# ming024/FastSpeech2

Measured on AMD Instinct MI355X. Metric: mel-frames/sec (train, 80-bin), higher is better.
Workload: dtype bf16; 1 GPU; BASELINE configs[1]: LJSpeech train, 4+4 FFT layers d=256 2 heads, 80-bin mel, batch=48/GPU, L=128 phonemes, T=925 frames, fwd+loss+bwd+clip+Adam, dropout on, fp32 master weights; global_batch=48, parallelism=dp1, hip_graph=False, side_stream_wgrad=True, windows=1, library=fastspeech2_amd/libfs2hip.so

## Files before the change

fastspeech2_amd/csrc/fs2_attn.hip:

```cpp
#include "fs2_common.h"
#include "fs2_gemm.h"
#include <type_traits>

typedef float f32x16 __attribute__((ext_vector_type(16)));

#define DK 128
__device__ __forceinline__ int swz(int row, int chunk) { return row * 512 + ((chunk ^ (row & 15)) << 4); }
__device__ __forceinline__ int crow(int r, int h2) { return (r & 3) + 8 * (r >> 2) + 4 * h2; }

template <typename T, int NT>
__device__ __forceinline__ void stage_tile(unsigned char* lds, const T* __restrict__ base, long ld, int row0, int nrows_valid,
                                           int tid) {
#pragma unroll
    for (int i = 0; i < 1024 / NT; ++i) {
        int idx = tid + NT * i;
        int r = idx >> 5, c = idx & 31;
        float4 v = make_float4(0.f, 0.f, 0.f, 0.f);
        if (r < nrows_valid) v = ld4<T>(base + (size_t)(row0 + r) * ld + c * 4);
        *reinterpret_cast<float4*>(lds + swz(r, c)) = v;
    }
}

template <typename T>
__global__ void __launch_bounds__(256, 1) attn_fwd_kernel(const T* __restrict__ qkv, long ld, T* __restrict__ ctx, long ldo,
                                                          float* __restrict__ lse, const int32_t* __restrict__ lens, int S,
                                                          int H, float scale) {
    __shared__ __attribute__((aligned(16))) unsigned char sK[32 * 512];
    __shared__ __attribute__((aligned(16))) unsigned char sV[32 * 512];
    const int tid = threadIdx.x, lane = tid & 63, w = tid >> 6, fl = lane & 31, h2 = lane >> 5;
    const int qt = blockIdx.x, h = blockIdx.y, b = blockIdx.z;
    const int len = lens ? min(lens[b], S) : S;
    const int q0 = qt * 128;
    const size_t rowbase = (size_t)b * S;
    T* out = ctx + rowbase * ldo + h * DK;
    float* lse_o = lse + ((size_t)b * H + h) * S;
    if (q0 >= len) {
        for (int i = tid; i < 128 * 32; i += 256) {
            int r = i >> 5, c = (i & 31) * 4;
            if (q0 + r < S) st4<T>(out + (size_t)(q0 + r) * ldo + c, make_float4(0.f, 0.f, 0.f, 0.f));
        }
        if (tid < 128 && q0 + tid < S) lse_o[q0 + tid] = 0.f;
        return;
    }
    const T* Q = qkv + rowbase * ld + h * DK;
    const T* K = qkv + rowbase * ld + (size_t)H * DK + h * DK;
    const T* V = qkv + rowbase * ld + (size_t)2 * H * DK + h * DK;

    const int myq = q0 + w * 32 + fl;
    float qf[64];
#pragma unroll
    for (int u = 0; u < 16; ++u) {
        float4 v = make_float4(0.f, 0.f, 0.f, 0.f);
        if (myq < S) v = ld4<T>(Q + (size_t)myq * ld + h2 * 64 + u * 4);
        qf[u * 4 + 0] = v.x * scale; qf[u * 4 + 1] = v.y * scale; qf[u * 4 + 2] = v.z * scale; qf[u * 4 + 3] = v.w * scale;
    }
    f32x16 o[4];
#pragma unroll
    for (int nb = 0; nb < 4; ++nb)
#pragma unroll
        for (int r = 0; r < 16; ++r) o[nb][r] = 0.f;
    float m = -INFINITY, l = 0.f;

    for (int k0 = 0; k0 < len; k0 += 32) {
        __syncthreads();
        stage_tile<T, 256>(sK, K, ld, k0, min(32, S - k0), tid);
        stage_tile<T, 256>(sV, V, ld, k0, min(32, S - k0), tid);
        __syncthreads();
        f32x16 s;
#pragma unroll
        for (int r = 0; r < 16; ++r) s[r] = 0.f;
#pragma unroll
        for (int u = 0; u < 16; ++u) {
            float4 kf = *reinterpret_cast<const float4*>(sK + swz(fl, h2 * 16 + u));
            s = __builtin_amdgcn_mfma_f32_32x32x2f32(kf.x, qf[u * 4 + 0], s, 0, 0, 0);
            s = __builtin_amdgcn_mfma_f32_32x32x2f32(kf.y, qf[u * 4 + 1], s, 0, 0, 0);
            s = __builtin_amdgcn_mfma_f32_32x32x2f32(kf.z, qf[u * 4 + 2], s, 0, 0, 0);
            s = __builtin_amdgcn_mfma_f32_32x32x2f32(kf.w, qf[u * 4 + 3], s, 0, 0, 0);
        }
        float mx = -INFINITY;
#pragma unroll
        for (int r = 0; r < 16; ++r) {
            if (k0 + crow(r, h2) >= len) s[r] = -INFINITY;
            mx = fmaxf(mx, s[r]);
        }
        mx = fmaxf(mx, __shfl_xor(mx, 32, 64));
        float mn = fmaxf(m, mx);
        float alpha = __expf(m - mn);
        float rs = 0.f;
#pragma unroll
        for (int r = 0; r < 16; ++r) { s[r] = __expf(s[r] - mn); rs += s[r]; }
        rs += __shfl_xor(rs, 32, 64);
        l = l * alpha + rs;
        m = mn;
#pragma unroll
        for (int r = 0; r < 16; ++r) {
            float ar = __shfl(alpha, crow(r, h2), 64);
#pragma unroll
            for (int nb = 0; nb < 4; ++nb) o[nb][r] *= ar;
        }
#pragma unroll
        for (int r = 0; r < 16; ++r) {
            int key = crow(r, h2);
#pragma unroll
            for (int nb = 0; nb < 4; ++nb) {
                int col = nb * 32 + fl;
                float vb = *reinterpret_cast<const float*>(sV + swz(key, col >> 2) + (col & 3) * 4);
                o[nb] = __builtin_amdgcn_mfma_f32_32x32x2f32(s[r], vb, o[nb], 0, 0, 0);
            }
        }
    }
    float linv = l > 0.f ? 1.f / l : 0.f;
    if (h2 == 0 && myq < S) lse_o[myq] = (l > 0.f) ? m + __logf(l) : 0.f;
#pragma unroll
    for (int r = 0; r < 16; ++r) {
        float li = __shfl(linv, crow(r, h2), 64);
        int q = q0 + w * 32 + crow(r, h2);
        if (q < S) {
#pragma unroll
            for (int nb = 0; nb < 4; ++nb) Elem<T>::st(out + (size_t)q * ldo + nb * 32 + fl, o[nb][r] * li);
        }
    }
}


typedef short s16x4 __attribute__((ext_vector_type(4)));
typedef short s16x8 __attribute__((ext_vector_type(8)));
typedef __bf16 bf16x8 __attribute__((ext_vector_type(8)));
typedef __attribute__((address_space(3))) s16x4* lds_s4p;

__device__ __forceinline__ int swzb(int row, int c16) { return row * 256 + ((c16 ^ (((row & 3) << 2) | ((row >> 2) & 3))) << 4); }

template <int NT, int ROWS>
__device__ __forceinline__ void stage_tile_bf16(unsigned char* lds, const bf16_t* __restrict__ base, long ld, int row0,
                                                int nrows_valid, int tid) {
#pragma unroll
    for (int i = 0; i < ROWS * 16 / NT; ++i) {
        int idx = tid + NT * i;
        int r = idx >> 4, c = idx & 15;
        uint4 v = make_uint4(0, 0, 0, 0);
        if (r < nrows_valid) v = *reinterpret_cast<const uint4*>(base + (size_t)(row0 + r) * ld + c * 8);
        *reinterpret_cast<uint4*>(lds + swzb(r, c)) = v;
    }
}
__device__ __forceinline__ bf16x8 frag_k(const unsigned char* lds, int row, int s, int h) {
    return __builtin_bit_cast(bf16x8, *reinterpret_cast<const uint4*>(lds + swzb(row, 2 * s + h)));
}
__device__ __forceinline__ bf16x8 frag_t(const unsigned char* lds, int rowbase, int nb, int lane) {
    int li = lane & 15, g = lane >> 4, h = g >> 1;
    int row = rowbase + 4 * h + (li >> 2);
    int col = nb * 32 + 16 * (g & 1) + 4 * (li & 3);
    int off0 = swzb(row, col >> 3) + ((col & 7) << 1);
    int off1 = swzb(row + 8, col >> 3) + ((col & 7) << 1);
    s16x4 lo = __builtin_amdgcn_ds_read_tr16_b64_v4i16((lds_s4p)(lds + off0));
    s16x4 hi = __builtin_amdgcn_ds_read_tr16_b64_v4i16((lds_s4p)(lds + off1));
    return __builtin_bit_cast(bf16x8, __builtin_shufflevector(lo, hi, 0, 1, 2, 3, 4, 5, 6, 7));
}
__device__ __forceinline__ bf16x8 pack8(const float* p) {
    uint4 v;
    v.x = pack_bf16x2(p[0], p[1]); v.y = pack_bf16x2(p[2], p[3]); v.z = pack_bf16x2(p[4], p[5]); v.w = pack_bf16x2(p[6], p[7]);
    return __builtin_bit_cast(bf16x8, v);
}
__device__ __forceinline__ void load_row_frags(bf16x8* f, const bf16_t* row, int h, bool ok) {
#pragma unroll
    for (int s = 0; s < 8; ++s) {
        uint4 v = make_uint4(0, 0, 0, 0);
        if (ok) v = *reinterpret_cast<const uint4*>(row + 16 * s + 8 * h);
        f[s] = __builtin_bit_cast(bf16x8, v);
    }
}

#define TILE_LD1(t, base, ld_, row0, last_row, I) \
    (t##I) = *reinterpret_cast<const uint4*>((base) + (unsigned)(min((row0) + ((tid + 256 * I) >> 4), (last_row)) * (int)(ld_) + (tid & 15) * 8))
#define TILE_LOAD_REGS(t, base, ld_, row0, last_row) do { TILE_LD1(t, base, ld_, row0, last_row, 0); TILE_LD1(t, base, ld_, row0, last_row, 1); \
    TILE_LD1(t, base, ld_, row0, last_row, 2); TILE_LD1(t, base, ld_, row0, last_row, 3); } while (0)
#define TILE_ST1(lds, t, I) *reinterpret_cast<uint4*>((lds) + swzb((tid + 256 * I) >> 4, tid & 15)) = (t##I)
#define TILE_STORE_REGS(lds, t) do { TILE_ST1(lds, t, 0); TILE_ST1(lds, t, 1); TILE_ST1(lds, t, 2); TILE_ST1(lds, t, 3); } while (0)


#ifdef FS2_DEV
__device__ unsigned long long fs2_attn_stamps[16 * 12];
__device__ int fs2_attn_stamp_kernel = 2;
extern "C" int fs2_dev_attn_stamp_select(int k) { return hipMemcpyToSymbol(HIP_SYMBOL(fs2_attn_stamp_kernel), &k, sizeof(int)) == hipSuccess ? 0 : 1; }
extern "C" int fs2_dev_attn_stamps(unsigned long long* out) {
    return hipMemcpyFromSymbol(out, HIP_SYMBOL(fs2_attn_stamps), sizeof(fs2_attn_stamps)) == hipSuccess ? 0 : 1;
}
#define FS2_STAMP_INIT() const bool fs2_stamp_on = fs2_attn_stamp_kernel == FS2_STAMP_KERNEL && blockIdx.x == 0 && blockIdx.y == 0 && blockIdx.z == 0 && threadIdx.x == 0
#define FS2_STAMP_AT(t0_, i) do { if (fs2_stamp_on && (t0_) < 16 * 64) fs2_attn_stamps[((t0_) >> 6) * 12 + (i)] = __builtin_amdgcn_s_memtime(); } while (0)
#define FS2_STAMP(i) FS2_STAMP_AT(q0, i)
#define FS2_STAMP_RAW(i) do { if (fs2_stamp_on) fs2_attn_stamps[(i)] = __builtin_amdgcn_s_memtime(); } while (0)
#else
#define FS2_STAMP_INIT() do {} while (0)
#define FS2_STAMP_AT(t0_, i) do {} while (0)
#define FS2_STAMP(i) do {} while (0)
#define FS2_STAMP_RAW(i) do {} while (0)
#endif

__device__ __forceinline__ void attn_block_map(int H, int& t, int& h, int& b) {
    const int nt = (int)gridDim.x, nbh = (int)(gridDim.y * gridDim.z);
    const int L = (int)(blockIdx.x + gridDim.x * (blockIdx.y + gridDim.y * blockIdx.z));
    const int G = L / (8 * nt), r = L - G * (8 * nt);
    const int rem = min(8, nbh - 8 * G);
    const int bh = 8 * G + r % rem;
    t = r / rem;
    b = bh / H; h = bh - b * H;
}

template <int IMG, int NTHR> struct FragAddrT {
    unsigned k[8], t0[4], t1[4], st[4];
    int step;
    __device__ __forceinline__ void init(unsigned base, int tid) {
        const int lane = tid & 63, fl = lane & 31, h2 = lane >> 5;
#pragma unroll
        for (int i = 0; i < 8; ++i) k[i] = base + (unsigned)swzb(fl, 2 * i + h2);
        const int li = lane & 15, g = lane >> 4, hh = g >> 1, rr = 4 * hh + (li >> 2);
#pragma unroll
        for (int nb = 0; nb < 4; ++nb) {
            const int col = nb * 32 + 16 * (g & 1) + 4 * (li & 3);
            t0[nb] = base + (unsigned)(swzb(rr, col >> 3) + ((col & 7) << 1));
            t1[nb] = base + (unsigned)(swzb(rr + 8, col >> 3) + ((col & 7) << 1));
        }
#pragma unroll
        for (int I = 0; I < 4; ++I) st[I] = base + (unsigned)(2 * IMG) + (unsigned)swzb((tid + NTHR * I) >> 4, tid & 15);
        step = 2 * IMG;
    }
    __device__ __forceinline__ void flip() {
#pragma unroll
        for (int i = 0; i < 8; ++i) k[i] += (unsigned)step;
#pragma unroll
        for (int nb = 0; nb < 4; ++nb) { t0[nb] += (unsigned)step; t1[nb] += (unsigned)step; }
#pragma unroll
        for (int I = 0; I < 4; ++I) st[I] -= (unsigned)step;
        step = -step;
    }
    __device__ __forceinline__ bf16x8 rk(int img, int blk, int i) const {
        typedef unsigned lds_v4u __attribute__((ext_vector_type(4)));
        typedef __attribute__((address_space(3))) const lds_v4u* lds_u4p;
        return __builtin_bit_cast(bf16x8, *(lds_u4p)(size_t)(k[i] + (unsigned)(img * IMG + blk * 8192)));
    }
    __device__ __forceinline__ bf16x8 rt(int img, int rb, int nb) const {
        s16x4 lo = __builtin_amdgcn_ds_read_tr16_b64_v4i16((lds_s4p)(size_t)(t0[nb] + (unsigned)(img * IMG + rb * 256)));
        s16x4 hi = __builtin_amdgcn_ds_read_tr16_b64_v4i16((lds_s4p)(size_t)(t1[nb] + (unsigned)(img * IMG + rb * 256)));
        return __builtin_bit_cast(bf16x8, __builtin_shufflevector(lo, hi, 0, 1, 2, 3, 4, 5, 6, 7));
    }
    __device__ __forceinline__ void store(int img, const uint4& v, int I) const {
#if defined(__HIP_DEVICE_COMPILE__)
        typedef unsigned lds_v4u __attribute__((ext_vector_type(4)));
        typedef __attribute__((address_space(3))) lds_v4u* lds_u4w;
        *(lds_u4w)(size_t)(st[I] + (unsigned)(img * IMG)) = lds_v4u{v.x, v.y, v.z, v.w};
#else
        (void)img; (void)v; (void)I;
#endif
    }
};
typedef FragAddrT<16384, 256> FragAddr;
#define TILE_STORE_FA(fa, img, t) do { (fa).store(img, t##0, 0); (fa).store(img, t##1, 1); (fa).store(img, t##2, 2); (fa).store(img, t##3, 3); } while (0)


typedef unsigned attn_u32x2 __attribute__((ext_vector_type(2)));
__device__ __forceinline__ void attn_store_row(bf16_t* rowp, const f32x16 (&acc)[4], float f, int h2, bool ok, bool live = true) {
#pragma unroll
    for (int nb = 0; nb < 4; ++nb) {
        float c[2][8];
#pragma unroll
        for (int e = 0; e < 4; ++e) {
            attn_u32x2 s0 = __builtin_amdgcn_permlane32_swap(__float_as_uint(acc[nb][e]), __float_as_uint(acc[nb][4 + e]), false, false);
            attn_u32x2 s1 = __builtin_amdgcn_permlane32_swap(__float_as_uint(acc[nb][8 + e]), __float_as_uint(acc[nb][12 + e]), false, false);
            c[0][e] = __uint_as_float(s0[0]); c[0][4 + e] = __uint_as_float(s0[1]);
            c[1][e] = __uint_as_float(s1[0]); c[1][4 + e] = __uint_as_float(s1[1]);
        }
        auto y = [&](float x) { return live ? x * f : 0.f; };
#pragma unroll
        for (int ch = 0; ch < 2; ++ch) {
            uint4 o;
            o.x = pack_bf16x2(y(c[ch][0]), y(c[ch][1])); o.y = pack_bf16x2(y(c[ch][2]), y(c[ch][3]));
            o.z = pack_bf16x2(y(c[ch][4]), y(c[ch][5])); o.w = pack_bf16x2(y(c[ch][6]), y(c[ch][7]));
            if (ok) *reinterpret_cast<uint4*>(rowp + nb * 32 + ch * 16 + h2 * 8) = o;
        }
    }
}

#define FS2_STAMP_KERNEL 0
__global__ void __launch_bounds__(256, 2) attn_fwd_bf16_kernel(const bf16_t* __restrict__ qkv, long ld, bf16_t* __restrict__ ctx,
                                                               long ldo, float* __restrict__ lse,
                                                               const int32_t* __restrict__ lens, int S, int H, float scale) {
    __shared__ __attribute__((aligned(16))) unsigned char sKV[2][2][64 * 256];
    FS2_STAMP_INIT();
    const int tid = threadIdx.x, lane = tid & 63, w = tid >> 6, fl = lane & 31, h2 = lane >> 5;
    int qt, h, b;
    attn_block_map(H, qt, h, b);
    const int len = lens ? min(lens[b], S) : S;
    const int q0 = qt * 128;
    const size_t rowbase = (size_t)b * S;
    bf16_t* out = ctx + rowbase * ldo + h * DK;
    float* lse_o = lse + ((size_t)b * H + h) * S;
    if (q0 >= len) {
        for (int i = tid; i < 128 * 32; i += 256) {
            int r = i >> 5, c = (i & 31) * 4;
            if (q0 + r < S) st4<bf16_t>(out + (size_t)(q0 + r) * ldo + c, make_float4(0.f, 0.f, 0.f, 0.f));
        }
        if (tid < 128 && q0 + tid < S) lse_o[q0 + tid] = 0.f;
        return;
    }
    const bf16_t* Q = qkv + rowbase * ld + h * DK;
    const bf16_t* K = qkv + rowbase * ld + (size_t)H * DK + h * DK;
    const bf16_t* V = qkv + rowbase * ld + (size_t)2 * H * DK + h * DK;
    const int myq = q0 + w * 32 + fl;
    bf16x8 qf[8];
    load_row_frags(qf, Q + (size_t)min(myq, S - 1) * ld, h2, myq < S);
    f32x16 o[4];
#pragma unroll
    for (int nb = 0; nb < 4; ++nb)
#pragma unroll
        for (int r = 0; r < 16; ++r) o[nb][r] = 0.f;
    float m = -INFINITY, l = 0.f;
    const float sc2 = scale * 1.4426950408889634f;

    uint4 tk0, tk1, tk2, tk3, tv0, tv1, tv2, tv3;
    TILE_LOAD_REGS(tk, K, ld, 0, S - 1);
    TILE_LOAD_REGS(tv, V, ld, 0, S - 1);
    TILE_STORE_REGS(sKV[0][0], tk);
    TILE_STORE_REGS(sKV[0][1], tv);
    __syncthreads();
    FragAddr fa;
    fa.init(lds_addr(&sKV[0][0][0]), tid);
    for (int k0 = 0; k0 < len; k0 += 64) {
        const bool more = k0 + 64 < len;
        FS2_STAMP_AT(k0, 0);
        if (more) {
            TILE_LOAD_REGS(tk, K, ld, k0 + 64, S - 1);
            TILE_LOAD_REGS(tv, V, ld, k0 + 64, S - 1);
        }
        FS2_STAMP_AT(k0, 1);
        f32x16 s[2];
#pragma unroll
        for (int kb = 0; kb < 2; ++kb)
#pragma unroll
            for (int r = 0; r < 16; ++r) s[kb][r] = 0.f;
        {
            __builtin_amdgcn_s_setprio(1);
            bf16x8 c0 = fa.rk(0, 0, 0), c1 = fa.rk(0, 1, 0);
#pragma unroll
            for (int st = 0; st < 8; ++st) {
                bf16x8 n0 = c0, n1 = c1;
                if (st < 7) { n0 = fa.rk(0, 0, st + 1); n1 = fa.rk(0, 1, st + 1); }
                __builtin_amdgcn_sched_barrier(0);
                s[0] = __builtin_amdgcn_mfma_f32_32x32x16_bf16(c0, qf[st], s[0], 0, 0, 0);
                s[1] = __builtin_amdgcn_mfma_f32_32x32x16_bf16(c1, qf[st], s[1], 0, 0, 0);
                __builtin_amdgcn_sched_barrier(0);
                c0 = n0; c1 = n1;
            }
            __builtin_amdgcn_s_setprio(0);
        }
        FS2_STAMP_AT(k0, 2);
        if (k0 + 64 > len) {
#pragma unroll
            for (int kb = 0; kb < 2; ++kb)
#pragma unroll
                for (int r = 0; r < 16; ++r)
                    if (k0 + kb * 32 + crow(r, h2) >= len) s[kb][r] = -INFINITY;
        }
        float mx = -INFINITY;
#pragma unroll
        for (int kb = 0; kb < 2; ++kb)
#pragma unroll
            for (int r = 0; r < 16; ++r) mx = fmaxf(mx, s[kb][r]);
        mx = fmaxf(mx, __shfl_xor(mx, 32, 64)) * sc2;
        if (__builtin_amdgcn_ballot_w64(mx > m + 8.f) != 0ull) {
            const float mn = fmaxf(m, mx);
            const float alpha = __builtin_amdgcn_exp2f(m - mn);
            l *= alpha;
            m = mn;
#pragma unroll
            for (int r = 0; r < 16; ++r) {
#pragma unroll
                for (int nb = 0; nb < 4; ++nb) o[nb][r] *= alpha;
            }
        }
        float rs = 0.f;
#pragma unroll
        for (int kb = 0; kb < 2; ++kb)
#pragma unroll
            for (int r = 0; r < 16; ++r) { s[kb][r] = __builtin_amdgcn_exp2f(fmaf(s[kb][r], sc2, -m)); rs += s[kb][r]; }
        rs += __shfl_xor(rs, 32, 64);
        l += rs;
        FS2_STAMP_AT(k0, 3);
        {
            bf16x8 cv[4], nv[4];
            __builtin_amdgcn_s_setprio(1);
#pragma unroll
            for (int nb = 0; nb < 4; ++nb) cv[nb] = fa.rt(1, 0, nb);
#pragma unroll
            for (int g = 0; g < 4; ++g) {
                if (g < 3) {
#pragma unroll
                    for (int nb = 0; nb < 4; ++nb) nv[nb] = fa.rt(1, 16 * (g + 1), nb);
                }
                float pv[8];
#pragma unroll
                for (int e = 0; e < 8; ++e) pv[e] = s[g >> 1][8 * (g & 1) + e];
                bf16x8 pa = pack8(pv);
                __builtin_amdgcn_sched_barrier(0);
#pragma unroll
                for (int nb = 0; nb < 4; ++nb) o[nb] = __builtin_amdgcn_mfma_f32_32x32x16_bf16(cv[nb], pa, o[nb], 0, 0, 0);
                __builtin_amdgcn_sched_barrier(0);
#pragma unroll
                for (int nb = 0; nb < 4; ++nb) cv[nb] = nv[nb];
            }
            __builtin_amdgcn_s_setprio(0);
        }
        FS2_STAMP_AT(k0, 4);
        if (more) {
            TILE_STORE_FA(fa, 0, tk);
            TILE_STORE_FA(fa, 1, tv);
        }
        fa.flip();
        FS2_STAMP_AT(k0, 5);
        __syncthreads();
        FS2_STAMP_AT(k0, 6);
    }
    float linv = l > 0.f ? 1.f / l : 0.f;
    if (h2 == 0 && myq < S) lse_o[myq] = (l > 0.f) ? m * 0.6931471805599453f + __logf(l) : 0.f;
    attn_store_row(out + (size_t)min(myq, S - 1) * ldo, o, linv, h2, myq < S);
}
#undef FS2_STAMP_KERNEL


#define FS2_SGB(mask, n) __builtin_amdgcn_sched_group_barrier((mask), (n), 0)
#define FS2_SG_MFMA 0x008
#define FS2_SG_VALU 0x002
#define FS2_SG_TRANS 0x400
#define FS2_SG_DSR 0x100
#define FS2_SG_DSW 0x200
#define FS2_STAMP_KERNEL 2
__global__ void __launch_bounds__(256, 1) attn_bwd_dkv2_bf16_kernel(const bf16_t* __restrict__ qkv, long ld,
                                                                    const bf16_t* __restrict__ dctx, long ldo,
                                                                    const float* __restrict__ lse, const float* __restrict__ delta,
                                                                    bf16_t* __restrict__ dqkv, const int32_t* __restrict__ lens,
                                                                    int S, int H, float scale) {
    __shared__ __attribute__((aligned(16))) unsigned char sQD[2][2][64 * 256];
    __shared__ __attribute__((aligned(16))) float sLD[2][2][64];
    FS2_STAMP_INIT();
    const int tid = threadIdx.x, lane = tid & 63, w = tid >> 6, fl = lane & 31, h2 = lane >> 5;
    int kt, h, b;
    attn_block_map(H, kt, h, b);
    const int len = lens ? min(lens[b], S) : S;
    const size_t rowbase = (size_t)b * S;
    const int kbase = kt * 128 + w * 32;
    bf16_t* dK = dqkv + rowbase * ld + (size_t)H * DK + h * DK;
    bf16_t* dV = dqkv + rowbase * ld + (size_t)2 * H * DK + h * DK;
    if (kt * 128 >= len) {
        for (int i = tid; i < 128 * 32; i += 256) {
            int r = i >> 5, c = (i & 31) * 4;
            if (kt * 128 + r < S) {
                st4<bf16_t>(dK + (size_t)(kt * 128 + r) * ld + c, make_float4(0.f, 0.f, 0.f, 0.f));
                st4<bf16_t>(dV + (size_t)(kt * 128 + r) * ld + c, make_float4(0.f, 0.f, 0.f, 0.f));
            }
        }
        return;
    }
    const bf16_t* Q = qkv + rowbase * ld + h * DK;
    const bf16_t* K = qkv + rowbase * ld + (size_t)H * DK + h * DK;
    const bf16_t* V = qkv + rowbase * ld + (size_t)2 * H * DK + h * DK;
    const bf16_t* dO = dctx + rowbase * ldo + h * DK;
    const float* lse_b = lse + ((size_t)b * H + h) * S;
    const float* del_b = delta + ((size_t)b * H + h) * S;
    const int mykey = kbase + fl;
    bf16x8 kf[8], vf[8];
    load_row_frags(kf, K + (size_t)min(mykey, S - 1) * ld, h2, mykey < S);
    load_row_frags(vf, V + (size_t)min(mykey, S - 1) * ld, h2, mykey < S);
    f32x16 dk[4], dv[4];
#pragma unroll
    for (int nb = 0; nb < 4; ++nb)
#pragma unroll
        for (int r = 0; r < 16; ++r) { dk[nb][r] = 0.f; dv[nb][r] = 0.f; }
    const float* ld_src = tid < 64 ? lse_b : del_b;
    const float sc2 = scale * 1.4426950408889634f;
    auto load_ld = [&](int q0) -> float {
        float v;
        const float* pa_ = ld_src + min(q0 + (tid & 63), S - 1);
        asm volatile("global_load_dword %0, %1, off" : "=v"(v) : "v"(pa_) : "memory");
        return v;
    };
    auto conv_ld = [&](float v, int q0) -> float {
        const int q = q0 + (tid & 63);
        if (tid < 64) v *= 1.4426950408889634f;
        if (q >= len) v = tid < 64 ? INFINITY : 0.f;
        return v;
    };
    const unsigned lds_qd = lds_addr(&sQD[0][0][0]);
    unsigned ak[8], at0[4], at1[4];
#pragma unroll
    for (int i = 0; i < 8; ++i) ak[i] = lds_qd + (unsigned)swzb(fl, 2 * i + h2);
    {
        const int li = lane & 15, g = lane >> 4, hh = g >> 1, rr = 4 * hh + (li >> 2);
#pragma unroll
        for (int nb = 0; nb < 4; ++nb) {
            const int col = nb * 32 + 16 * (g & 1) + 4 * (li & 3);
            at0[nb] = lds_qd + (unsigned)(swzb(rr, col >> 3) + ((col & 7) << 1));
            at1[nb] = lds_qd + (unsigned)(swzb(rr + 8, col >> 3) + ((col & 7) << 1));
        }
    }
    typedef __attribute__((address_space(3))) const uint4* lds_u4p;
    auto rdk = [&](int arr, int qb, int i) -> bf16x8 {
        return __builtin_bit_cast(bf16x8, *(lds_u4p)(size_t)(ak[i] + (unsigned)(arr * 16384 + qb * 8192)));
    };
    auto rdt = [&](int arr, int rb, int nb) -> bf16x8 {
        s16x4 lo = __builtin_amdgcn_ds_read_tr16_b64_v4i16((lds_s4p)(size_t)(at0[nb] + (unsigned)(arr * 16384 + rb * 256)));
        s16x4 hi = __builtin_amdgcn_ds_read_tr16_b64_v4i16((lds_s4p)(size_t)(at1[nb] + (unsigned)(arr * 16384 + rb * 256)));
        return __builtin_bit_cast(bf16x8, __builtin_shufflevector(lo, hi, 0, 1, 2, 3, 4, 5, 6, 7));
    };
    unsigned voq[4], vod[4];
    int prow[4];
#pragma unroll
    for (int j = 0; j < 4; ++j) {
        const int row = 4 * (w + 4 * j) + (lane >> 4);
        const int c = (lane & 15) ^ (((row & 3) << 2) | ((row >> 2) & 3));
        prow[j] = row;
        voq[j] = (unsigned)c * 16u; vod[j] = (unsigned)c * 16u;
    }
    auto dma_piece = [&](int q0, int buf, int j) {
        const unsigned r = (unsigned)min(q0 + prow[j], S - 1);
        const unsigned dst = __builtin_amdgcn_readfirstlane(lds_qd + (unsigned)(buf * 32768 + (w + 4 * j) * 1024));
        glds16_sbase(r * (unsigned)(ld * 2) + voq[j], Q, dst);
        glds16_sbase(r * (unsigned)(ldo * 2) + vod[j], dO, dst + 16384u);
    };
    auto dma_tile = [&](int q0, int buf) {
#pragma unroll
        for (int j = 0; j < 4; ++j) dma_piece(q0, buf, j);
    };
    float tl = 0.f;
    dma_tile(0, 0);
    tl = load_ld(0);
    asm volatile("s_waitcnt vmcnt(0)" : "+v"(tl) :: "memory");
    if (tid < 128) sLD[0][tid >> 6][tid & 63] = conv_ld(tl, 0);
    __syncthreads();

    auto softmax8 = [&](const f32x16& s, const f32x16& dp, const float* sl, const float* sd, int qb, int u, bf16x8& pa, bf16x8& da) {
        float4 l4[2], d4[2];
#pragma unroll
        for (int g = 0; g < 2; ++g) {
            l4[g] = *reinterpret_cast<const float4*>(sl + qb * 32 + 8 * (2 * u + g) + 4 * h2);
            d4[g] = *reinterpret_cast<const float4*>(sd + qb * 32 + 8 * (2 * u + g) + 4 * h2);
        }
        float pv[8], dsv[8];
#pragma unroll
        for (int e = 0; e < 8; ++e) {
            const float lq = reinterpret_cast<const float*>(&l4[e >> 2])[e & 3];
            const float dq_ = reinterpret_cast<const float*>(&d4[e >> 2])[e & 3];
            const float p = __builtin_amdgcn_exp2f(fmaf(s[8 * u + e], sc2, -lq));
            pv[e] = p;
            dsv[e] = p * (dp[8 * u + e] - dq_);
        }
        pa = pack8(pv); da = pack8(dsv);
    };

#define FS2_PIN_ACC() asm volatile("" : "+a"(dk[0]), "+a"(dk[1]), "+a"(dk[2]), "+a"(dk[3]), "+a"(dv[0]), "+a"(dv[1]), "+a"(dv[2]), "+a"(dv[3]))
#pragma unroll
    for (int i = 0; i < 8; ++i) asm volatile("" : "+v"(kf[i]), "+v"(vf[i]));
    int buf = 0, flip = 32768;
    for (int q0 = 0; q0 < len; q0 += 64, buf ^= 1) {
        const bool more = q0 + 64 < len;
        FS2_STAMP(0);
        constexpr int sQ = 0, sdO = 1;
        const float* sl = sLD[buf][0];
        const float* sd = sLD[buf][1];
        bf16x8 x0q[4], x0d[4], y0q[4], y0d[4], x1q[4], x1d[4], y1q[4], y1d[4];
        bf16x8 t0d[4], t0q[4], u0d[4], u0q[4], t1d[4], t1q[4], u1d[4], u1q[4];
        f32x16 s0, p0, s1, p1;
        bf16x8 pa0a, da0a, pa0b, da0b, pa1a, da1a, pa1b, da1b;
#pragma unroll
        for (int i = 0; i < 4; ++i) { x0q[i] = rdk(sQ, 0, i); x0d[i] = rdk(sdO, 0, i); }
#pragma unroll
        for (int i = 0; i < 4; ++i) { y0q[i] = rdk(sQ, 0, 4 + i); y0d[i] = rdk(sdO, 0, 4 + i); }
        tl = load_ld(q0 + 64);
#pragma unroll
        for (int r = 0; r < 16; ++r) { s0[r] = 0.f; p0[r] = 0.f; }
        FS2_PIN_ACC(); __builtin_amdgcn_sched_barrier(0);
#pragma unroll
        for (int i = 0; i < 4; ++i) {
            s0 = __builtin_amdgcn_mfma_f32_32x32x16_bf16(x0q[i], kf[i], s0, 0, 0, 0);
            p0 = __builtin_amdgcn_mfma_f32_32x32x16_bf16(x0d[i], vf[i], p0, 0, 0, 0);
            x1q[i] = rdk(sQ, 1, i); x1d[i] = rdk(sdO, 1, i);
            if ((i & 1) && more) dma_piece(q0 + 64, buf ^ 1, i >> 1);
            __builtin_amdgcn_sched_barrier(0);
        }
        FS2_STAMP(1);
#pragma unroll
        for (int i = 0; i < 4; ++i) {
            s0 = __builtin_amdgcn_mfma_f32_32x32x16_bf16(y0q[i], kf[4 + i], s0, 0, 0, 0);
            p0 = __builtin_amdgcn_mfma_f32_32x32x16_bf16(y0d[i], vf[4 + i], p0, 0, 0, 0);
            y1q[i] = rdk(sQ, 1, 4 + i); y1d[i] = rdk(sdO, 1, 4 + i);
            if ((i & 1) && more) dma_piece(q0 + 64, buf ^ 1, 2 + (i >> 1));
            __builtin_amdgcn_sched_barrier(0);
        }
#pragma unroll
        for (int r = 0; r < 16; ++r) { s1[r] = 0.f; p1[r] = 0.f; }
        FS2_PIN_ACC(); __builtin_amdgcn_sched_barrier(0);
        FS2_STAMP(2);
#pragma unroll
        for (int i = 0; i < 4; ++i) {
            s1 = __builtin_amdgcn_mfma_f32_32x32x16_bf16(x1q[i], kf[i], s1, 0, 0, 0);
            p1 = __builtin_amdgcn_mfma_f32_32x32x16_bf16(x1d[i], vf[i], p1, 0, 0, 0);
        }
        softmax8(s0, p0, sl, sd, 0, 0, pa0a, da0a);
#pragma unroll
        for (int nb = 0; nb < 4; ++nb) { t0d[nb] = rdt(sdO, 0, nb); t0q[nb] = rdt(sQ, 0, nb); }
#pragma unroll
        for (int k = 0; k < 8; ++k) { FS2_SGB(FS2_SG_MFMA, 1); FS2_SGB(FS2_SG_DSR, 2); FS2_SGB(FS2_SG_VALU, 6); FS2_SGB(FS2_SG_TRANS, 1); }
        FS2_PIN_ACC(); __builtin_amdgcn_sched_barrier(0);
        FS2_STAMP(3);
#pragma unroll
        for (int i = 0; i < 4; ++i) {
            s1 = __builtin_amdgcn_mfma_f32_32x32x16_bf16(y1q[i], kf[4 + i], s1, 0, 0, 0);
            p1 = __builtin_amdgcn_mfma_f32_32x32x16_bf16(y1d[i], vf[4 + i], p1, 0, 0, 0);
        }
        softmax8(s0, p0, sl, sd, 0, 1, pa0b, da0b);
#pragma unroll
        for (int nb = 0; nb < 4; ++nb) { u0d[nb] = rdt(sdO, 16, nb); u0q[nb] = rdt(sQ, 16, nb); }
#pragma unroll
        for (int k = 0; k < 8; ++k) { FS2_SGB(FS2_SG_MFMA, 1); FS2_SGB(FS2_SG_DSR, 2); FS2_SGB(FS2_SG_VALU, 6); FS2_SGB(FS2_SG_TRANS, 1); }
        FS2_PIN_ACC(); __builtin_amdgcn_sched_barrier(0);
        FS2_STAMP(4);
#pragma unroll
        for (int nb = 0; nb < 4; ++nb) {
            dv[nb] = __builtin_amdgcn_mfma_f32_32x32x16_bf16(t0d[nb], pa0a, dv[nb], 0, 0, 0);
            dk[nb] = __builtin_amdgcn_mfma_f32_32x32x16_bf16(t0q[nb], da0a, dk[nb], 0, 0, 0);
        }
        softmax8(s1, p1, sl, sd, 1, 0, pa1a, da1a);
#pragma unroll
        for (int nb = 0; nb < 4; ++nb) { t1d[nb] = rdt(sdO, 32, nb); t1q[nb] = rdt(sQ, 32, nb); }
#pragma unroll
        for (int k = 0; k < 8; ++k) { FS2_SGB(FS2_SG_MFMA, 1); FS2_SGB(FS2_SG_DSR, 2); FS2_SGB(FS2_SG_VALU, 6); FS2_SGB(FS2_SG_TRANS, 1); }
        FS2_PIN_ACC(); __builtin_amdgcn_sched_barrier(0);
        FS2_STAMP(5);
#pragma unroll
        for (int nb = 0; nb < 4; ++nb) {
            dv[nb] = __builtin_amdgcn_mfma_f32_32x32x16_bf16(u0d[nb], pa0b, dv[nb], 0, 0, 0);
            dk[nb] = __builtin_amdgcn_mfma_f32_32x32x16_bf16(u0q[nb], da0b, dk[nb], 0, 0, 0);
        }
        softmax8(s1, p1, sl, sd, 1, 1, pa1b, da1b);
#pragma unroll
        for (int nb = 0; nb < 4; ++nb) { u1d[nb] = rdt(sdO, 48, nb); u1q[nb] = rdt(sQ, 48, nb); }
#pragma unroll
        for (int k = 0; k < 8; ++k) { FS2_SGB(FS2_SG_MFMA, 1); FS2_SGB(FS2_SG_DSR, 2); FS2_SGB(FS2_SG_VALU, 6); FS2_SGB(FS2_SG_TRANS, 1); }
        FS2_PIN_ACC(); __builtin_amdgcn_sched_barrier(0);
        FS2_STAMP(6);
#pragma unroll
        for (int nb = 0; nb < 4; ++nb) {
            dv[nb] = __builtin_amdgcn_mfma_f32_32x32x16_bf16(t1d[nb], pa1a, dv[nb], 0, 0, 0);
            dk[nb] = __builtin_amdgcn_mfma_f32_32x32x16_bf16(t1q[nb], da1a, dk[nb], 0, 0, 0);
        }
#pragma unroll
        for (int nb = 0; nb < 4; ++nb) {
            dv[nb] = __builtin_amdgcn_mfma_f32_32x32x16_bf16(u1d[nb], pa1b, dv[nb], 0, 0, 0);
            dk[nb] = __builtin_amdgcn_mfma_f32_32x32x16_bf16(u1q[nb], da1b, dk[nb], 0, 0, 0);
        }
        FS2_STAMP(7);
        asm volatile("s_waitcnt vmcnt(0)" : "+v"(tl) :: "memory");
        FS2_STAMP(8);
        if (tid < 128) sLD[buf ^ 1][tid >> 6][tid & 63] = conv_ld(tl, q0 + 64);
#pragma unroll
        for (int i = 0; i < 8; ++i) ak[i] += (unsigned)flip;
#pragma unroll
        for (int nb = 0; nb < 4; ++nb) { at0[nb] += (unsigned)flip; at1[nb] += (unsigned)flip; }
        flip = -flip;
        FS2_PIN_ACC();
        FS2_STAMP(9);
        __syncthreads();
        FS2_STAMP(10);
    }
    attn_store_row(dK + (size_t)min(mykey, S - 1) * ld, dk, scale, h2, mykey < S, mykey < len);
    attn_store_row(dV + (size_t)min(mykey, S - 1) * ld, dv, 1.f, h2, mykey < S, mykey < len);
}
#undef FS2_STAMP_KERNEL
#define FS2_STAMP_KERNEL 1
__global__ void __launch_bounds__(256, 2) attn_bwd_dq_bf16_kernel(const bf16_t* __restrict__ qkv, long ld,
                                                                  const bf16_t* __restrict__ ctx,
                                                                  const bf16_t* __restrict__ dctx, long ldo,
                                                                  const float* __restrict__ lse, float* __restrict__ delta,
                                                                  bf16_t* __restrict__ dqkv, const int32_t* __restrict__ lens,
                                                                  int S, int H, float scale) {
    __shared__ __attribute__((aligned(16))) unsigned char sKV[2][2][64 * 256];
    FS2_STAMP_INIT();
    FS2_STAMP_RAW(0);
    const int tid = threadIdx.x, lane = tid & 63, w = tid >> 6, fl = lane & 31, h2 = lane >> 5;
    int qt, h, b;
    attn_block_map(H, qt, h, b);
    const int len = lens ? min(lens[b], S) : S;
    const int q0 = qt * 128;
    const size_t rowbase = (size_t)b * S;
    bf16_t* dQ = dqkv + rowbase * ld + h * DK;
    if (q0 >= len) {
        for (int i = tid; i < 128 * 32; i += 256) {
            int r = i >> 5, c = (i & 31) * 4;
            if (q0 + r < S) st4<bf16_t>(dQ + (size_t)(q0 + r) * ld + c, make_float4(0.f, 0.f, 0.f, 0.f));
        }
        if (tid < 128 && q0 + tid < S) delta[((size_t)b * H + h) * S + q0 + tid] = 0.f;
        return;
    }
    const bf16_t* Q = qkv + rowbase * ld + h * DK;
    const bf16_t* K = qkv + rowbase * ld + (size_t)H * DK + h * DK;
    const bf16_t* V = qkv + rowbase * ld + (size_t)2 * H * DK + h * DK;
    const bf16_t* dO = dctx + rowbase * ldo + h * DK;
    const int myq = q0 + w * 32 + fl;
    const bool q_ok = myq < len;
    float my_lse = 0.f, my_del = 0.f;
    if (myq < S) my_lse = lse[((size_t)b * H + h) * S + myq];
    const float sc2 = scale * 1.4426950408889634f;
    const float my_lse2 = q_ok ? my_lse * 1.4426950408889634f : INFINITY;
    bf16x8 qf[8], df[8];
    load_row_frags(qf, Q + (size_t)min(myq, S - 1) * ld, h2, myq < S);
    load_row_frags(df, dO + (size_t)min(myq, S - 1) * ldo, h2, myq < S);
    {
        bf16x8 of[8];
        load_row_frags(of, ctx + (rowbase + (size_t)min(myq, S - 1)) * ldo + h * DK, h2, myq < S);
        float acc = 0.f;
#pragma unroll
        for (int st = 0; st < 8; ++st) {
            const uint4 ov = __builtin_bit_cast(uint4, of[st]), dv_ = __builtin_bit_cast(uint4, df[st]);
            const uint32_t* ou = reinterpret_cast<const uint32_t*>(&ov);
            const uint32_t* du = reinterpret_cast<const uint32_t*>(&dv_);
#pragma unroll
            for (int e = 0; e < 4; ++e)
                acc += __uint_as_float(ou[e] << 16) * __uint_as_float(du[e] << 16) + __uint_as_float(ou[e] & 0xffff0000u) * __uint_as_float(du[e] & 0xffff0000u);
        }
        acc += __shfl_xor(acc, 32, 64);
        my_del = acc;
        if (h2 == 0 && myq < S) delta[((size_t)b * H + h) * S + myq] = my_del;
    }
    f32x16 dq[4];
#pragma unroll
    for (int nb = 0; nb < 4; ++nb)
#pragma unroll
        for (int r = 0; r < 16; ++r) dq[nb][r] = 0.f;

    uint4 tk0, tk1, tk2, tk3, tv0, tv1, tv2, tv3;
    TILE_LOAD_REGS(tk, K, ld, 0, S - 1);
    TILE_LOAD_REGS(tv, V, ld, 0, S - 1);
    TILE_STORE_REGS(sKV[0][0], tk);
    TILE_STORE_REGS(sKV[0][1], tv);
    __syncthreads();
    FragAddr fa;
    fa.init(lds_addr(&sKV[0][0][0]), tid);
    FS2_STAMP_RAW(1);
    for (int k0 = 0; k0 < len; k0 += 64) {
        const bool more = k0 + 64 < len;
        FS2_STAMP_AT(k0 + 64, 0);
        if (more) {
            TILE_LOAD_REGS(tk, K, ld, k0 + 64, S - 1);
            TILE_LOAD_REGS(tv, V, ld, k0 + 64, S - 1);
        }
        FS2_STAMP_AT(k0 + 64, 1);
#pragma unroll
        for (int kb = 0; kb < 2; ++kb) {
            if (k0 + kb * 32 >= len) break;
            f32x16 s, dp;
#pragma unroll
            for (int r = 0; r < 16; ++r) { s[r] = 0.f; dp[r] = 0.f; }
            {
                __builtin_amdgcn_s_setprio(1);
                bf16x8 ck = fa.rk(0, kb, 0), cv = fa.rk(1, kb, 0);
#pragma unroll
                for (int st = 0; st < 8; ++st) {
                    bf16x8 nk = ck, nv = cv;
                    if (st < 7) { nk = fa.rk(0, kb, st + 1); nv = fa.rk(1, kb, st + 1); }
                    __builtin_amdgcn_sched_barrier(0);
                    s = __builtin_amdgcn_mfma_f32_32x32x16_bf16(ck, qf[st], s, 0, 0, 0);
                    dp = __builtin_amdgcn_mfma_f32_32x32x16_bf16(cv, df[st], dp, 0, 0, 0);
                    __builtin_amdgcn_sched_barrier(0);
                    ck = nk; cv = nv;
                }
                __builtin_amdgcn_s_setprio(0);
            }
            FS2_STAMP_AT(k0 + 64, 2 + 3 * kb);
            float dsv[16];
            if (k0 + kb * 32 + 32 > len) {
                int thr = len - k0 - kb * 32 - 4 * h2;
                asm volatile("" : "+v"(thr));
#pragma unroll
                for (int r = 0; r < 16; ++r)
                    if ((r & 3) + 8 * (r >> 2) >= thr) s[r] = -INFINITY;
            }
#pragma unroll
            for (int r = 0; r < 16; ++r) {
                const float p = __builtin_amdgcn_exp2f(fmaf(s[r], sc2, -my_lse2));
                dsv[r] = p * (dp[r] - my_del);
            }
            FS2_STAMP_AT(k0 + 64, 3 + 3 * kb);
            __builtin_amdgcn_s_setprio(1);
#pragma unroll
            for (int u = 0; u < 2; ++u) {
                bf16x8 da = pack8(dsv + 8 * u);
#pragma unroll
                for (int nb = 0; nb < 4; ++nb)
                    dq[nb] = __builtin_amdgcn_mfma_f32_32x32x16_bf16(fa.rt(0, kb * 32 + 16 * u, nb), da, dq[nb], 0, 0, 0);
            }
            __builtin_amdgcn_s_setprio(0);
            FS2_STAMP_AT(k0 + 64, 4 + 3 * kb);
        }
        if (more) {
            TILE_STORE_FA(fa, 0, tk);
            TILE_STORE_FA(fa, 1, tv);
        }
        fa.flip();
        FS2_STAMP_AT(k0 + 64, 8);
        __syncthreads();
        FS2_STAMP_AT(k0 + 64, 9);
    }
    attn_store_row(dQ + (size_t)min(myq, S - 1) * ld, dq, scale, h2, myq < S);
}
#undef FS2_STAMP_KERNEL

extern "C" int fs2_attn_fwd(const void* qkv, void* ctx, float* lse, const int32_t* lens, int B, int S, int H, int dk,
                            float scale, int dtype, hipStream_t stream) {
    FS2_CHECK_ARG(qkv && ctx && lse, "attn_fwd: null pointer");
    FS2_CHECK_ARG(dk == DK, "attn_fwd: only d_k = 128 is supported (got %d)", dk);
    FS2_CHECK_ARG(B >= 0 && S > 0 && H > 0, "attn_fwd: bad shape");
    if (B == 0) return FS2_OK;
    dim3 grid(fs2_cdiv(S, 128), H, B);
    long ld = 3L * H * DK, ldo = (long)H * DK;
    if (dtype == FS2_F32) attn_fwd_kernel<float><<<grid, 256, 0, stream>>>((const float*)qkv, ld, (float*)ctx, ldo, lse, lens, S, H, scale);
    else if (dtype == FS2_BF16) attn_fwd_bf16_kernel<<<grid, 256, 0, stream>>>((const bf16_t*)qkv, ld, (bf16_t*)ctx, ldo, lse, lens, S, H, scale);
    else { fs2_set_error("attn_fwd: dtype"); return FS2_EDTYPE; }
    FS2_CHECK_LAUNCH("attn_fwd");
    return FS2_OK;
}

template <typename T>
__global__ void attn_delta_kernel(const T* __restrict__ ctx, const T* __restrict__ dctx, float* __restrict__ delta, int rows,
                                  int S, int H) {
    int idx = blockIdx.x * (blockDim.x >> 6) + (threadIdx.x >> 6);
    if (idx >= rows * H) return;
    int lane = threadIdx.x & 63;
    int row = idx / H, h = idx - row * H;
    size_t off = (size_t)row * H * DK + h * DK + lane * 2;
    float s = Elem<T>::ld(ctx + off) * Elem<T>::ld(dctx + off) + Elem<T>::ld(ctx + off + 1) * Elem<T>::ld(dctx + off + 1);
    s = wave_sum(s);
    if (lane == 0) {
        int b = row / S, q = row - b * S;
        delta[((size_t)b * H + h) * S + q] = s;
    }
}

template <typename T>
__global__ void __launch_bounds__(256, 1) attn_bwd_dkv_kernel(const T* __restrict__ qkv, long ld, const T* __restrict__ dctx,
                                                              long ldo, const float* __restrict__ lse,
                                                              const float* __restrict__ delta, T* __restrict__ dqkv,
                                                              const int32_t* __restrict__ lens, int S, int H, float scale) {
    extern __shared__ __attribute__((aligned(16))) unsigned char smem[];
    const int tid = threadIdx.x, lane = tid & 63, w = tid >> 6, fl = lane & 31, h2 = lane >> 5;
    const int kt = blockIdx.x, h = blockIdx.y, b = blockIdx.z;
    const int len = lens ? min(lens[b], S) : S;
    const size_t rowbase = (size_t)b * S;
    const int kbase = kt * 128 + w * 32;
    T* dK = dqkv + rowbase * ld + (size_t)H * DK + h * DK;
    T* dV = dqkv + rowbase * ld + (size_t)2 * H * DK + h * DK;
    if (kt * 128 >= len) {
        for (int i = tid; i < 128 * 32; i += 256) {
            int r = i >> 5, c = (i & 31) * 4;
            if (kt * 128 + r < S) {
                st4<T>(dK + (size_t)(kt * 128 + r) * ld + c, make_float4(0.f, 0.f, 0.f, 0.f));
                st4<T>(dV + (size_t)(kt * 128 + r) * ld + c, make_float4(0.f, 0.f, 0.f, 0.f));
            }
        }
        return;
    }
    unsigned char* sKw = smem + w * 32768;
    unsigned char* sVw = sKw + 16384;
    unsigned char* sQ = smem + 131072;
    unsigned char* sdO = sQ + 16384;
    const T* Q = qkv + rowbase * ld + h * DK;
    const T* K = qkv + rowbase * ld + (size_t)H * DK + h * DK;
    const T* V = qkv + rowbase * ld + (size_t)2 * H * DK + h * DK;
    const T* dO = dctx + rowbase * ldo + h * DK;
    const float* lse_b = lse + ((size_t)b * H + h) * S;
    const float* del_b = delta + ((size_t)b * H + h) * S;
    stage_tile<T, 64>(sKw, K, ld, kbase, max(0, min(32, S - kbase)), lane);
    stage_tile<T, 64>(sVw, V, ld, kbase, max(0, min(32, S - kbase)), lane);
    const bool key_ok = (kbase + fl) < len;

    f32x16 dk[4], dv[4];
#pragma unroll
    for (int nb = 0; nb < 4; ++nb)
#pragma unroll
        for (int r = 0; r < 16; ++r) { dk[nb][r] = 0.f; dv[nb][r] = 0.f; }

    for (int q0 = 0; q0 < len; q0 += 32) {
        __syncthreads();
        stage_tile<T, 256>(sQ, Q, ld, q0, min(32, S - q0), tid);
        stage_tile<T, 256>(sdO, dO, ldo, q0, min(32, S - q0), tid);
        __syncthreads();
        f32x16 s, dp;
#pragma unroll
        for (int r = 0; r < 16; ++r) { s[r] = 0.f; dp[r] = 0.f; }
#pragma unroll
        for (int u = 0; u < 16; ++u) {
            float4 qa = *reinterpret_cast<const float4*>(sQ + swz(fl, h2 * 16 + u));
            float4 kb = *reinterpret_cast<const float4*>(sKw + swz(fl, h2 * 16 + u));
            s = __builtin_amdgcn_mfma_f32_32x32x2f32(qa.x, kb.x, s, 0, 0, 0);
            s = __builtin_amdgcn_mfma_f32_32x32x2f32(qa.y, kb.y, s, 0, 0, 0);
            s = __builtin_amdgcn_mfma_f32_32x32x2f32(qa.z, kb.z, s, 0, 0, 0);
            s = __builtin_amdgcn_mfma_f32_32x32x2f32(qa.w, kb.w, s, 0, 0, 0);
        }
#pragma unroll
        for (int u = 0; u < 16; ++u) {
            float4 da = *reinterpret_cast<const float4*>(sdO + swz(fl, h2 * 16 + u));
            float4 vb = *reinterpret_cast<const float4*>(sVw + swz(fl, h2 * 16 + u));
            dp = __builtin_amdgcn_mfma_f32_32x32x2f32(da.x, vb.x, dp, 0, 0, 0);
            dp = __builtin_amdgcn_mfma_f32_32x32x2f32(da.y, vb.y, dp, 0, 0, 0);
            dp = __builtin_amdgcn_mfma_f32_32x32x2f32(da.z, vb.z, dp, 0, 0, 0);
            dp = __builtin_amdgcn_mfma_f32_32x32x2f32(da.w, vb.w, dp, 0, 0, 0);
        }
#pragma unroll
        for (int r = 0; r < 16; ++r) {
            int q = q0 + crow(r, h2);
            float p = 0.f, ds = 0.f;
            if (key_ok && q < len) {
                p = __expf(s[r] * scale - lse_b[q]);
                ds = p * (dp[r] - del_b[q]) * scale;
            }
            s[r] = p; dp[r] = ds;
        }
#pragma unroll
        for (int r = 0; r < 16; ++r) {
            int qr = crow(r, h2);
#pragma unroll
            for (int nb = 0; nb < 4; ++nb) {
                int col = nb * 32 + fl;
                float ob = *reinterpret_cast<const float*>(sdO + swz(qr, col >> 2) + (col & 3) * 4);
                float qb = *reinterpret_cast<const float*>(sQ + swz(qr, col >> 2) + (col & 3) * 4);
                dv[nb] = __builtin_amdgcn_mfma_f32_32x32x2f32(s[r], ob, dv[nb], 0, 0, 0);
                dk[nb] = __builtin_amdgcn_mfma_f32_32x32x2f32(dp[r], qb, dk[nb], 0, 0, 0);
            }
        }
    }
#pragma unroll
    for (int r = 0; r < 16; ++r) {
        int key = kbase + crow(r, h2);
        if (key < S) {
#pragma unroll
            for (int nb = 0; nb < 4; ++nb) {
                Elem<T>::st(dK + (size_t)key * ld + nb * 32 + fl, dk[nb][r]);
                Elem<T>::st(dV + (size_t)key * ld + nb * 32 + fl, dv[nb][r]);
            }
        }
    }
}

template <typename T>
__global__ void __launch_bounds__(256, 1) attn_bwd_dq_kernel(const T* __restrict__ qkv, long ld, const T* __restrict__ dctx,
                                                             long ldo, const float* __restrict__ lse,
                                                             const float* __restrict__ delta, T* __restrict__ dqkv,
                                                             const int32_t* __restrict__ lens, int S, int H, float scale) {
    __shared__ __attribute__((aligned(16))) unsigned char sK[32 * 512];
    __shared__ __attribute__((aligned(16))) unsigned char sV[32 * 512];
    const int tid = threadIdx.x, lane = tid & 63, w = tid >> 6, fl = lane & 31, h2 = lane >> 5;
    const int qt = blockIdx.x, h = blockIdx.y, b = blockIdx.z;
// ... 108 lines not shown
```

Measured before the change: 4.613 million mel-frames/s.

## Load K/V tiles directly into LDS via global-to-LDS DMA in attention kernels

Replaces the register-staged K/V tile prefetch (global load into VGPRs, then ds_write into the swizzled LDS buffer) with direct global-to-LDS loads (glds16_sbase) into the alternate double buffer, in both the forward and dQ backward attention kernels. The swizzle is now applied on the global-read side through a per-lane XOR offset, and a vmcnt(0) wait is placed before each barrier. This removes eight uint4 staging registers and the LDS store instructions, which lowers VGPR pressure and frees issue slots. In exchange it relies on the DMA swizzle mapping matching the fragment readers. It also adds asm barriers to keep the q/dO fragments resident, and makes the lse load unconditional by clamping its index.

```diff
diff --git a/fastspeech2_amd/csrc/fs2_attn.hip b/fastspeech2_amd/csrc/fs2_attn.hip
--- a/fastspeech2_amd/csrc/fs2_attn.hip
+++ b/fastspeech2_amd/csrc/fs2_attn.hip
@@ -163,18 +163,11 @@
 __device__ __forceinline__ void load_row_frags(bf16x8* f, const bf16_t* row, int h, bool ok) {
 #pragma unroll
     for (int s = 0; s < 8; ++s) {
-        uint4 v = make_uint4(0, 0, 0, 0);
-        if (ok) v = *reinterpret_cast<const uint4*>(row + 16 * s + 8 * h);
-        f[s] = __builtin_bit_cast(bf16x8, v);
-    }
-}
-
-#define TILE_LD1(t, base, ld_, row0, last_row, I) \
-    (t##I) = *reinterpret_cast<const uint4*>((base) + (unsigned)(min((row0) + ((tid + 256 * I) >> 4), (last_row)) * (int)(ld_) + (tid & 15) * 8))
-#define TILE_LOAD_REGS(t, base, ld_, row0, last_row) do { TILE_LD1(t, base, ld_, row0, last_row, 0); TILE_LD1(t, base, ld_, row0, last_row, 1); \
-    TILE_LD1(t, base, ld_, row0, last_row, 2); TILE_LD1(t, base, ld_, row0, last_row, 3); } while (0)
-#define TILE_ST1(lds, t, I) *reinterpret_cast<uint4*>((lds) + swzb((tid + 256 * I) >> 4, tid & 15)) = (t##I)
-#define TILE_STORE_REGS(lds, t) do { TILE_ST1(lds, t, 0); TILE_ST1(lds, t, 1); TILE_ST1(lds, t, 2); TILE_ST1(lds, t, 3); } while (0)
+        const uint4 v = *reinterpret_cast<const uint4*>(row + 16 * s + 8 * h);
+        f[s] = __builtin_bit_cast(bf16x8, ok ? v : make_uint4(0, 0, 0, 0));
+    }
+}
+
 
 
 #ifdef FS2_DEV
@@ -205,8 +198,8 @@
     b = bh / H; h = bh - b * H;
 }
 
-template <int IMG, int NTHR> struct FragAddrT {
-    unsigned k[8], t0[4], t1[4], st[4];
+template <int IMG> struct FragAddrT {
+    unsigned k[8], t0[4], t1[4];
     int step;
     __device__ __forceinline__ void init(unsigned base, int tid) {
         const int lane = tid & 63, fl = lane & 31, h2 = lane >> 5;
@@ -219,8 +212,6 @@
             t0[nb] = base + (unsigned)(swzb(rr, col >> 3) + ((col & 7) << 1));
             t1[nb] = base + (unsigned)(swzb(rr + 8, col >> 3) + ((col & 7) << 1));
         }
-#pragma unroll
-        for (int I = 0; I < 4; ++I) st[I] = base + (unsigned)(2 * IMG) + (unsigned)swzb((tid + NTHR * I) >> 4, tid & 15);
         step = 2 * IMG;
     }
     __device__ __forceinline__ void flip() {
@@ -228,8 +219,6 @@
         for (int i = 0; i < 8; ++i) k[i] += (unsigned)step;
 #pragma unroll
         for (int nb = 0; nb < 4; ++nb) { t0[nb] += (unsigned)step; t1[nb] += (unsigned)step; }
-#pragma unroll
-        for (int I = 0; I < 4; ++I) st[I] -= (unsigned)step;
         step = -step;
     }
     __device__ __forceinline__ bf16x8 rk(int img, int blk, int i) const {
@@ -242,18 +231,29 @@
         s16x4 hi = __builtin_amdgcn_ds_read_tr16_b64_v4i16((lds_s4p)(size_t)(t1[nb] + (unsigned)(img * IMG + rb * 256)));
         return __builtin_bit_cast(bf16x8, __builtin_shufflevector(lo, hi, 0, 1, 2, 3, 4, 5, 6, 7));
     }
-    __device__ __forceinline__ void store(int img, const uint4& v, int I) const {
-#if defined(__HIP_DEVICE_COMPILE__)
-        typedef unsigned lds_v4u __attribute__((ext_vector_type(4)));
-        typedef __attribute__((address_space(3))) lds_v4u* lds_u4w;
-        *(lds_u4w)(size_t)(st[I] + (unsigned)(img * IMG)) = lds_v4u{v.x, v.y, v.z, v.w};
-#else
-        (void)img; (void)v; (void)I;
-#endif
-    }
 };
-typedef FragAddrT<16384, 256> FragAddr;
-#define TILE_STORE_FA(fa, img, t) do { (fa).store(img, t##0, 0); (fa).store(img, t##1, 1); (fa).store(img, t##2, 2); (fa).store(img, t##3, 3); } while (0)
+typedef FragAddrT<16384> FragAddr;
+
+struct KvDma {
+    unsigned vo, lds0;
+    int prow, w;
+    __device__ __forceinline__ void init(unsigned lds_base, int tid) {
+        const int lane = tid & 63;
+        w = tid >> 6;
+        prow = 4 * w + (lane >> 4);
+        vo = (unsigned)((lane & 15) ^ (((lane >> 4) << 2) | w)) * 16u;
+        lds0 = lds_base + (unsigned)(w * 1024);
+    }
+    __device__ __forceinline__ void tile(const bf16_t* K, const bf16_t* V, long ld, int row0, int last_row, unsigned bufoff) const {
+#pragma unroll
+        for (int j = 0; j < 4; ++j) {
+            const unsigned off = (unsigned)min(row0 + prow + 16 * j, last_row) * (unsigned)(ld * 2) + vo;
+            const unsigned dst = __builtin_amdgcn_readfirstlane(lds0 + bufoff + (unsigned)(j * 4096));
+            glds16_sbase(off, K, dst);
+            glds16_sbase(off, V, dst + 16384u);
+        }
+    }
+};
 
 
 typedef unsigned attn_u32x2 __attribute__((ext_vector_type(2)));
@@ -315,21 +315,20 @@
     float m = -INFINITY, l = 0.f;
     const float sc2 = scale * 1.4426950408889634f;
 
-    uint4 tk0, tk1, tk2, tk3, tv0, tv1, tv2, tv3;
-    TILE_LOAD_REGS(tk, K, ld, 0, S - 1);
-    TILE_LOAD_REGS(tv, V, ld, 0, S - 1);
-    TILE_STORE_REGS(sKV[0][0], tk);
-    TILE_STORE_REGS(sKV[0][1], tv);
-    __syncthreads();
     FragAddr fa;
     fa.init(lds_addr(&sKV[0][0][0]), tid);
-    for (int k0 = 0; k0 < len; k0 += 64) {
+    KvDma dma;
+    dma.init(lds_addr(&sKV[0][0][0]), tid);
+    dma.tile(K, V, ld, 0, S - 1, 0u);
+    asm volatile("s_waitcnt vmcnt(0)" ::: "memory");
+#pragma unroll
+    for (int i = 0; i < 8; ++i) asm volatile("" : "+v"(qf[i]));
+    __syncthreads();
+    unsigned nbuf = 32768u;
+    for (int k0 = 0; k0 < len; k0 += 64, nbuf ^= 32768u) {
         const bool more = k0 + 64 < len;
         FS2_STAMP_AT(k0, 0);
-        if (more) {
-            TILE_LOAD_REGS(tk, K, ld, k0 + 64, S - 1);
-            TILE_LOAD_REGS(tv, V, ld, k0 + 64, S - 1);
-        }
+        if (more) dma.tile(K, V, ld, k0 + 64, S - 1, nbuf);
         FS2_STAMP_AT(k0, 1);
         f32x16 s[2];
 #pragma unroll
@@ -409,11 +408,8 @@
             __builtin_amdgcn_s_setprio(0);
         }
         FS2_STAMP_AT(k0, 4);
-        if (more) {
-            TILE_STORE_FA(fa, 0, tk);
-            TILE_STORE_FA(fa, 1, tv);
-        }
         fa.flip();
+        asm volatile("s_waitcnt vmcnt(0)" ::: "memory");
         FS2_STAMP_AT(k0, 5);
         __syncthreads();
         FS2_STAMP_AT(k0, 6);
@@ -704,8 +700,8 @@
     const bf16_t* dO = dctx + rowbase * ldo + h * DK;
     const int myq = q0 + w * 32 + fl;
     const bool q_ok = myq < len;
-    float my_lse = 0.f, my_del = 0.f;
-    if (myq < S) my_lse = lse[((size_t)b * H + h) * S + myq];
+    float my_lse, my_del = 0.f;
+    my_lse = lse[((size_t)b * H + h) * S + min(myq, S - 1)];
     const float sc2 = scale * 1.4426950408889634f;
     const float my_lse2 = q_ok ? my_lse * 1.4426950408889634f : INFINITY;
     bf16x8 qf[8], df[8];
@@ -734,22 +730,21 @@
 #pragma unroll
         for (int r = 0; r < 16; ++r) dq[nb][r] = 0.f;
 
-    uint4 tk0, tk1, tk2, tk3, tv0, tv1, tv2, tv3;
-    TILE_LOAD_REGS(tk, K, ld, 0, S - 1);
-    TILE_LOAD_REGS(tv, V, ld, 0, S - 1);
-    TILE_STORE_REGS(sKV[0][0], tk);
-    TILE_STORE_REGS(sKV[0][1], tv);
-    __syncthreads();
     FragAddr fa;
     fa.init(lds_addr(&sKV[0][0][0]), tid);
+    KvDma dma;
+    dma.init(lds_addr(&sKV[0][0][0]), tid);
+    dma.tile(K, V, ld, 0, S - 1, 0u);
+    asm volatile("s_waitcnt vmcnt(0)" ::: "memory");
+#pragma unroll
+    for (int i = 0; i < 8; ++i) asm volatile("" : "+v"(qf[i]), "+v"(df[i]));
+    __syncthreads();
     FS2_STAMP_RAW(1);
-    for (int k0 = 0; k0 < len; k0 += 64) {
+    unsigned nbuf = 32768u;
+    for (int k0 = 0; k0 < len; k0 += 64, nbuf ^= 32768u) {
         const bool more = k0 + 64 < len;
         FS2_STAMP_AT(k0 + 64, 0);
-        if (more) {
-            TILE_LOAD_REGS(tk, K, ld, k0 + 64, S - 1);
-            TILE_LOAD_REGS(tv, V, ld, k0 + 64, S - 1);
-        }
+        if (more) dma.tile(K, V, ld, k0 + 64, S - 1, nbuf);
         FS2_STAMP_AT(k0 + 64, 1);
 #pragma unroll
         for (int kb = 0; kb < 2; ++kb) {
@@ -798,11 +793,8 @@
             __builtin_amdgcn_s_setprio(0);
             FS2_STAMP_AT(k0 + 64, 4 + 3 * kb);
         }
-        if (more) {
-            TILE_STORE_FA(fa, 0, tk);
-            TILE_STORE_FA(fa, 1, tv);
-        }
         fa.flip();
+        asm volatile("s_waitcnt vmcnt(0)" ::: "memory");
         FS2_STAMP_AT(k0 + 64, 8);
         __syncthreads();
         FS2_STAMP_AT(k0 + 64, 9);
```

After: 4.631 million mel-frames/s (median of 6 runs). Within noise of the previous version (+0.4%).
